# mkangquantum/quits

Hardware: AMD Instinct MI355X
Metric: decoded shots/sec + logical-error-rate, [[144,12,12]] BB code, d rounds, p=0.003 (higher is better)
Workload: dtype f32

## Files before the change

### include/quits_amd.h

```cpp
#ifndef QUITS_AMD_H
#define QUITS_AMD_H

#include <stdint.h>

#ifdef __cplusplus
extern "C" {
#endif

#define QD_OK 0
#define QD_EINVAL (-1)
#define QD_EUNSUPPORTED (-2)
#define QD_EHIP (-3)
#define QD_ECAPACITY (-4)

#define QD_BP_PRODUCT_SUM 0
#define QD_BP_MINIMUM_SUM 1
#define QD_SCHEDULE_PARALLEL 0
#define QD_SCHEDULE_SERIAL 1
#define QD_OSD_OFF 0
#define QD_OSD_0 1
#define QD_OSD_E 2
#define QD_OSD_CS 3
#define QD_LSD_0 4
#define QD_LSD_E 5
// ... 27 lines not shown
} qd_params;

int qd_version(void);
const char *qd_last_error(void);
int qd_device_count(void);

int qd_graph_create(int32_t m, int32_t n, const int32_t *row_ptr, const int32_t *col_idx, const double *priors,
                    int32_t device, qd_graph **out);
void qd_graph_destroy(qd_graph *g);
int qd_graph_info(const qd_graph *g, int32_t *info);
int qd_graph_info_ex(const qd_graph *g, int32_t *info, int32_t n_entries);

int qd_decoder_create(const qd_graph *g, const qd_params *params, qd_decoder **out);
void qd_decoder_destroy(qd_decoder *d);
int qd_decoder_info(const qd_decoder *d, int32_t *info);
#define QD_POST_NONE 0
#define QD_POST_OSD0_SR 1
#define QD_POST_OSD0_REG 2
#define QD_POST_OSD_W_OLD 3
#define QD_POST_OSD_CS_PANEL 4
#define QD_POST_LSD 5
int qd_decoder_postproc_kernel(const qd_decoder *d);
int qd_decoder_reserve(qd_decoder *d, int64_t max_batch);
int qd_decoder_set_workspace_limit(qd_decoder *d, int64_t bytes);
int qd_decoder_release_workspace(qd_decoder *d);

int qd_decode_batch(qd_decoder *d, const uint8_t *d_det, int64_t det_stride, int64_t det_offset,
                    const uint8_t *d_upd, int64_t upd_stride, int32_t upd_rows, int64_t B,
                    uint32_t *d_err_bits, int32_t *d_status, void *stream);

// ... 44 lines not shown
```

### quits_amd/_lib.py

```python
from __future__ import annotations

import ctypes as C
import os

_HERE = os.path.dirname(os.path.abspath(__file__))
LIB_PATH = os.environ.get("QUITS_AMD_LIB", os.path.join(_HERE, "lib", "libquits_amd.so"))

QD_BP = {"product_sum": 0, "ps": 0, "prod_sum": 0, "minimum_sum": 1, "min_sum": 1, "ms": 1, 0: 0, 1: 1}
QD_SCHEDULE = {"parallel": 0, "p": 0, "serial": 1, "s": 1, 0: 0, 1: 1}
QD_OSD = {"osd_off": 0, "off": 0, "osd_0": 1, "osd0": 1, "osd_e": 2, "osde": 2, "exhaustive": 2,
          "osd_cs": 3, "osdcs": 3, "combination_sweep": 3, "lsd_0": 4, "lsd_e": 5, "lsd_cs": 6, 0: 0, 1: 1, 2: 2, 3: 3, 4: 4, 5: 5, 6: 6}

STATUS_ITER_MASK = 0x3FFF
STATUS_COARSE_GRID = 1 << 14
STATUS_INEXACT = 1 << 15
STATUS_CONVERGED = 1 << 16
STATUS_OSD = 1 << 17
STATUS_INCONSISTENT = 1 << 18
STATUS_ZERO = 1 << 19


class QdParams(C.Structure):
    _fields_ = [("bp_method", C.c_int32), ("schedule", C.c_int32), ("max_iter", C.c_int32),
                ("osd_method", C.c_int32), ("osd_order", C.c_int32), ("reserved", C.c_int32),
                ("ms_scaling_factor", C.c_double)]


class QdError(RuntimeError):
    def __init__(self, code, msg):
        super().__init__("libquits_amd error %d: %s" % (code, msg))
        self.code = code


_lib = None

EXPORTS = [
    "qd_version", "qd_last_error", "qd_device_count", "qd_graph_create", "qd_graph_destroy", "qd_graph_info", "qd_graph_info_ex",
    "qd_decoder_create", "qd_decoder_info", "qd_decoder_postproc_kernel", "qd_decoder_destroy", "qd_decoder_reserve", "qd_decoder_set_workspace_limit", "qd_decoder_release_workspace", "qd_decode_batch", "qd_decode_stage", "qd_osd0_batch", "qd_decoder_failed_llr",
    "qd_decoder_set_profiling", "qd_decoder_profile", "qd_decoder_post_head_start", "qd_decoder_debug_counters", "qd_spmat_create", "qd_spmat_destroy", "qd_gf2_spmv_batch",
    "qd_unpack_bits", "qd_count_mismatch", "qd_sample_dem",
    "qd_circuit_create", "qd_circuit_destroy", "qd_circuit_info", "qd_sample_circuit",
]


def load():
    global _lib
    if _lib is not None:
        return _lib
    if not os.path.exists(LIB_PATH):
        raise RuntimeError(
            "quits_amd: %s is missing -- build it with `python -c 'import __graft_entry__ as g; g.build()'` "
            "(hipcc --offload-arch=gfx950).  There is no CPU fallback." % LIB_PATH)
    try:
# ... 4 lines not shown
    vp, i32, i64, u64 = C.c_void_p, C.c_int32, C.c_int64, C.c_uint64
    L.qd_version.restype = C.c_int
    if L.qd_version() < 104:
        raise RuntimeError("quits_amd: %s is version %d, this package needs >= 104 -- rebuild it (`python -c 'import __graft_entry__ as g; g.build()'`)"
                           % (LIB_PATH, L.qd_version()))
    L.qd_last_error.restype = C.c_char_p
    L.qd_device_count.restype = C.c_int
    L.qd_graph_create.argtypes = [i32, i32, vp, vp, vp, i32, C.POINTER(vp)]
    L.qd_graph_destroy.argtypes = [vp]
    L.qd_graph_destroy.restype = None
    L.qd_graph_info.argtypes = [vp, vp]
    L.qd_graph_info_ex.argtypes = [vp, vp, i32]
    L.qd_decoder_create.argtypes = [vp, C.POINTER(QdParams), C.POINTER(vp)]
    L.qd_decoder_info.argtypes = [vp, vp]
    L.qd_decoder_postproc_kernel.argtypes = [vp]
    L.qd_decoder_postproc_kernel.restype = C.c_int
    L.qd_decoder_destroy.argtypes = [vp]
    L.qd_decoder_destroy.restype = None
    L.qd_decoder_reserve.argtypes = [vp, i64]
    L.qd_decoder_set_workspace_limit.argtypes = [vp, i64]
    L.qd_decoder_release_workspace.argtypes = [vp]
    L.qd_decode_batch.argtypes = [vp, vp, i64, i64, vp, i64, i32, i64, vp, vp, vp]
    L.qd_decode_stage.argtypes = [vp, vp, i64, i64, vp, i64, i32, i64, vp, vp, i32, vp]
    L.qd_osd0_batch.argtypes = [vp, vp, i64, i64, vp, i64, i32, i64, vp, vp, vp, vp]
    L.qd_decoder_failed_llr.argtypes = [vp, i64, vp, vp]
    L.qd_decoder_set_profiling.argtypes = [vp, i32]
    L.qd_decoder_post_head_start.argtypes = [vp, i32, vp]
    L.qd_decoder_profile.argtypes = [vp, vp, i32]
    L.qd_decoder_debug_counters.argtypes = [vp, vp]
    L.qd_spmat_create.argtypes = [i32, i32, vp, vp, i32, C.POINTER(vp)]
# ... 28 lines not shown
```

### quits_amd/csrc/bp_scatter_edge.h

```cpp
#pragma once
#include "qd_internal.h"
#include <float.h>

__device__ __forceinline__ float qs_min_abs(float a, float b)
{
    float r;
    asm("v_min_f32 %0, %1, |%2|" : "=v"(r) : "v"(a), "v"(b));
    return r;
}
typedef uint32_t qs_u32x4 __attribute__((ext_vector_type(4)));
__device__ __forceinline__ uint4 qs_as_uint4(qs_u32x4 v) { return make_uint4(v.x, v.y, v.z, v.w); }
typedef __attribute__((address_space(3))) int32_t qs_lds_i32;
#define QS_LDS(off) ((qs_lds_i32 *)(uintptr_t)(uint32_t)(off))
#define QS_BIG 1.0e30f
#ifndef QS_PRIO
#define QS_PRIO 1
#endif

#define QS_SIGN31(sb) (((sgnw >> (sb)) & 1u) << 31)
#define QS_HP1(A_) hp ^= (uint32_t)(A_);
#define QS_HPA(A_) hpa = (uint32_t)(A_);
#define QS_HPB(A_) hp = __builtin_amdgcn_bitop3_b32(hp, hpa, (uint32_t)(A_), 0x96);
#define QS_EDGE(off, k_, sb, TAILFIX) QS_EDGE_H(off, k_, sb, TAILFIX, QS_HP1)
#define QS_EDGE_H(off, k_, sb, TAILFIX, HP)                                                                  \
    {                                                                                                        \
        const int A_ = *QS_LDS(QS_ADDR(off));                                                                \
        const float mag_ = ((uint32_t)(k_) == kold) ? s2 : s1;                                               \
        const float prev_ = __uint_as_float(QS_SIGN31(sb) | __float_as_uint(mag_));                          \
        float d_ = (float)A_ - prev_;                                                                        \
        TAILFIX(d_, k_)                                                                                      \
        const float bm_ = d_ + 1.0f;                                                                         \
        HP(A_)                                                                                               \
        neww = __builtin_amdgcn_alignbit(neww, __float_as_uint(d_), 31);                                     \
                   \
        asm("v_cmp_lt_f32 vcc, |%1|, %2\n\tv_addc_co_u32 %0, vcc, %0, %0, vcc" : "+v"(ltw) : "v"(bm_), "v"(a1) : "vcc"); \
        a2 = __builtin_amdgcn_fmed3f(a1, a2, fabsf(bm_));                                                    \
        a1 = qs_min_abs(a1, bm_);                                                                            \
    }
#define QS_NOFIX(x_, k_)
#define QS_TAILFIX(x_, k_) x_ = ((int)(k_) < dc) ? x_ : QS_BIG;

// ... 30 lines not shown
```

### quits_amd/csrc/bp_scatter_wide.hip

```cpp
#include "qd_internal.h"
#include "../../include/quits_amd.h"
#include "bp_scatter_edge.h"

#ifndef QSW_SCAT_SGPR_POS
#define QSW_SCAT_SGPR_POS 1
#endif
#ifndef QSW_GPRIO
#define QSW_GPRIO 1
#endif
#ifndef QSW_PRIO_BASE
#define QSW_PRIO_BASE 0
#endif

__device__ __forceinline__ uint4 qs_reuse4(uint4 &v) { asm volatile("" : "+v"(v.x), "+v"(v.y), "+v"(v.z), "+v"(v.w)); return v; }

template <int T, int MW, int CPL, int NSW>
__global__ void __launch_bounds__(T, MW) qd_bp_scatter_wide_kernel(BpGraphDev g, ScatGraphDev sg, DecodeArgs a, ScatArgs x)
{
    extern __shared__ __align__(16) unsigned char smem[];
    const uint32_t lds_base = (uint32_t)(uintptr_t)(__attribute__((address_space(3))) unsigned char *)smem;
    if (lds_base != 0u) __builtin_trap();
    uint32_t *outw = reinterpret_cast<uint32_t *>(smem + sg.off_out);
    int *misc = reinterpret_cast<int *>(smem + sg.off_misc);
    constexpr int NW = T / 64;
// ... 60 lines not shown
    const __amdgpu_buffer_rsrc_t adj_rsrc = __builtin_amdgcn_make_buffer_rsrc((void *)sg.adjA, 0, (g.max_rdeg_pad / 4 + 2) * m_pad * 16, 0x00020000);
    const int adj_row = m_pad * 16;
#define QS_ADJ_LOAD(row_) qs_as_uint4(__builtin_amdgcn_raw_buffer_load_b128(adj_rsrc, adj_voff, (row_) * adj_row, 0))
#ifdef QS_ABL_NOADJ
#define QS_ADJ(row_) qs_reuse4(adjc)
#define QS_ABL_ADJC uint4 adjc = QS_ADJ_LOAD(0);
#else
#define QS_ADJ(row_) QS_ADJ_LOAD(row_)
#define QS_ABL_ADJC
#endif
#ifndef QSW_PREFETCH
#define QSW_PREFETCH 1
#endif
#define QS_ADJ_FIRST qs_as_uint4(__builtin_amdgcn_raw_buffer_load_b128(adj_rsrc, cs[0] * 16, 0, 0))
    uint4 pf = QS_ADJ_FIRST;
    int t = 0, converged = 0;
    for (;;) {
        bool us = false;
#pragma unroll
        for (int j = 0; j < CPL; ++j) {
            float a1 = FLT_MAX, a2 = FLT_MAX;
            uint32_t kst = 0u;
#if QSW_GPRIO
            if (j == 0) __builtin_amdgcn_s_setprio(QSW_PRIO_BASE); else if (j == CPL - 1) __builtin_amdgcn_s_setprio((QSW_PRIO_BASE + 2) & 3); else __builtin_amdgcn_s_setprio((QSW_PRIO_BASE + 1) & 3);
#endif
            if (act[j]) {
                int dwj = dws[j];
                asm volatile("" : "+s"(dwj));
                const int trip = dwj & 0xFF, wmax = (dwj >> 8) & 0xFF, wmin = (dwj >> 16) & 0xFF, wmin4 = wmin & ~3;
                const int adj_voff = cs[j] * 16;
                QS_ABL_ADJC
                const float s1 = S1[j], s2 = S2[j];
                const uint32_t kold = KOLD[j];
                const int dc = dcs[j];
                uint32_t hp = 0u, hpa = 0u, par = 0u;
                uint32_t neg[NSW];
#pragma unroll
                for (int w = 0; w < NSW; ++w) {
                    neg[w] = 0u;
                    const int k0 = 32 * w;
                    if (k0 < trip) {
                        const uint32_t sgnw = O[j][w];
                        uint32_t neww = 0u, ltw = 0u;
                        const int kend = min(trip - k0, 32);
                        const int kplain = min(max(wmin4 - k0, 0), kend);
                        const int row0 = k0 >> 2;
                        uint4 nx = (QSW_PREFETCH && j == 0 && w == 0) ? pf : QS_ADJ(row0);
                        int kk = 0;
                        {
                            uint4 eb;
#pragma unroll 1
                            for (; kk + 8 <= kplain; kk += 8) {
                                eb = QS_ADJ(row0 + (kk >> 2) + 1);
                                {
                                    const int sb = kend - 1 - kk, k = k0 + kk;
                                    QS_EDGE_H(nx.x, k, sb, QS_NOFIX, QS_HPA) QS_EDGE_H(nx.y, k + 1, sb - 1, QS_NOFIX, QS_HPB)
                                    QS_EDGE_H(nx.z, k + 2, sb - 2, QS_NOFIX, QS_HPA) QS_EDGE_H(nx.w, k + 3, sb - 3, QS_NOFIX, QS_HPB)
                                }
                                nx = QS_ADJ(row0 + (kk >> 2) + 2);
                                {
                                    const int sb = kend - 5 - kk, k = k0 + kk + 4;
                                    QS_EDGE_H(eb.x, k, sb, QS_NOFIX, QS_HPA) QS_EDGE_H(eb.y, k + 1, sb - 1, QS_NOFIX, QS_HPB)
                                    QS_EDGE_H(eb.z, k + 2, sb - 2, QS_NOFIX, QS_HPA) QS_EDGE_H(eb.w, k + 3, sb - 3, QS_NOFIX, QS_HPB)
                                }
                            }
                        }
#pragma unroll 1
                        for (; kk < kplain; kk += 4) {
                            const uint4 e4 = nx;
                            nx = QS_ADJ(row0 + (kk >> 2) + 1);
                            const int sb = kend - 1 - kk, k = k0 + kk;
                            QS_EDGE_H(e4.x, k, sb, QS_NOFIX, QS_HPA)
                            QS_EDGE_H(e4.y, k + 1, sb - 1, QS_NOFIX, QS_HPB)
                            QS_EDGE_H(e4.z, k + 2, sb - 2, QS_NOFIX, QS_HPA)
                            QS_EDGE_H(e4.w, k + 3, sb - 3, QS_NOFIX, QS_HPB)
                        }
#define QS_TAIL_EDGE(off, q_)                                                                                     \
                            if (k + (q_) < wmin) QS_EDGE(off, k + (q_), sb - (q_), QS_NOFIX)                      \
                            else if (k + (q_) < wmax) QS_EDGE(off, k + (q_), sb - (q_), QS_TAILFIX)               \
                            else { neww <<= 1; ltw <<= 1; }
#pragma unroll 1
                        for (; kk + 4 < kend; kk += 4) {
                            const uint4 e4 = nx;
                            nx = QS_ADJ(row0 + (kk >> 2) + 1);
                            const int sb = kend - 1 - kk, k = k0 + kk;
                            QS_TAIL_EDGE(e4.x, 0) QS_TAIL_EDGE(e4.y, 1) QS_TAIL_EDGE(e4.z, 2) QS_TAIL_EDGE(e4.w, 3)
                        }
                        if (kk < kend) {
                            const int sb = kend - 1 - kk, k = k0 + kk;
                            QS_TAIL_EDGE(nx.x, 0) QS_TAIL_EDGE(nx.y, 1) QS_TAIL_EDGE(nx.z, 2) QS_TAIL_EDGE(nx.w, 3)
                        }
#undef QS_TAIL_EDGE
                        neg[w] = neww;
                        par ^= neww;
                        if (ltw) kst = (uint32_t)(k0 + kend - 1 - (int)__builtin_ctz(ltw));
                    }
                }
                const uint32_t flip = 0u - ((synd[j] ^ (uint32_t)__popc(par)) & 1u);
#pragma unroll
                for (int w = 0; w < NSW; ++w) Q[j][w] = neg[w] ^ flip;
                mx2 = fmaxf(mx2, a2);
                us = us || (((synd[j] ^ (hp >> 31)) & 1u) != 0u);
            }
            A1[j] = a1; A2[j] = a2; KST[j] = kst;
        }
#if QSW_GPRIO
        __builtin_amdgcn_s_setprio(QSW_PRIO_BASE);
#endif
        if (QSW_PREFETCH) pf = QS_ADJ_FIRST;
        {
            const unsigned long long bal = __ballot(us);
            if ((tid & 63) == 0) misc[32 + (tid >> 6)] = (bal != 0ull);
        }
        __syncthreads();
        int anyun = 0;
        {
            const int4 *f4 = reinterpret_cast<const int4 *>(misc + 32);
            for (int w = 0; w < (NW + 3) / 4; ++w) {
                const int4 v = f4[w];
                anyun |= v.x | v.y | v.z | v.w;
            }
        }
#ifndef QS_ABL_FORCE_ITERS
        if (t >= 1 && !anyun) { converged = 1; break; }
#endif
        if (t == a.max_iter) break;
        __builtin_amdgcn_s_setprio((QSW_PRIO_BASE + QS_PRIO) & 3);
#pragma unroll
        for (int j = 0; j < CPL; ++j) {
#ifdef QSW_STATS
            {
                bool same = A1[j] == S1[j] && A2[j] == S2[j] && (KST[j] == KOLD[j] || A1[j] == A2[j]);
#pragma unroll
                for (int w = 0; w < NSW; ++w) same = same && Q[j][w] == O[j][w];
                const unsigned long long ba = __ballot(act[j]), bs = __ballot(act[j] && same);
                if ((tid & 63) == 0 && ba) {
                    const int bk = min(t / 10, 4);
                    atomicAdd(&a.dbg[0], 1ull); atomicAdd(&a.dbg[2 + bk], 1ull);
                    if (bs == ba) { atomicAdd(&a.dbg[1], 1ull); atomicAdd(&a.dbg[7 + bk], 1ull); }
                    atomicAdd(&a.dbg[12], (unsigned long long)__popcll(bs)); atomicAdd(&a.dbg[13], (unsigned long long)__popcll(ba));
                }
// ... 84 lines not shown
                    const int vn = sg_ ? -dlt : dlt;
                    (void)__hip_atomic_fetch_add(QS_LDS(fixn_off), vn, __ATOMIC_RELAXED, __HIP_MEMORY_SCOPE_WORKGROUP);
                    (void)__hip_atomic_fetch_add(QS_LDS(FOFF[j]), -FVAL[j], __ATOMIC_RELAXED, __HIP_MEMORY_SCOPE_WORKGROUP);
                    FOFF[j] = fixn_off; FVAL[j] = vn;
                }
            }
            S1[j] = A1[j]; S2[j] = A2[j]; KOLD[j] = KST[j];
#pragma unroll
            for (int w = 0; w < NSW; ++w) O[j][w] = Q[j][w];
        }
        __builtin_amdgcn_s_setprio(QSW_PRIO_BASE);
        if (QSW_PREFETCH) pf = QS_ADJ_FIRST;
        __syncthreads();
        ++t;
    }
#undef QS_ADJ
#undef QS_ADJ_FIRST
#undef QS_ADJ_LOAD
#undef QS_ABL_ADJC

    {
        const int tripped = qd_block_or(!(mx2 < x.m2_limit) ? 1 : 0, misc, NW, 0);
        if (tripped) {
            if (tid == 0) {
                const int at = atomicAdd(x.recheck_count, 1);
                if (at < x.recheck_cap) x.recheck_list[at] = (int32_t)shot;
            }
            return;
        }
    }
    for (int b = tid; b < sg.nslots; b += T)
        if (*QS_LDS(cur + 4u * (uint32_t)b) < 0) {
            const uint32_t jf = sg.slot_fault[b];
            if (jf != 0xFFFFFFFFu) atomicOr(&outw[jf >> 5], 1u << (jf & 31u));
        }
    if (!converged && a.want_llr && tid == 0) misc[48] = atomicAdd(a.fail_count, 1);
    __syncthreads();
    for (int w = tid; w < g.out_words; w += T) a.err_bits[shot * g.out_words + w] = outw[w];
    if (!converged && a.want_llr) {
        const int slot = misc[48];
        float *dst = a.llr_ws + (int64_t)slot * n_pad;
        for (int k1 = tid; k1 < g.n; k1 += T) dst[k1] = (float)(*QS_LDS(cur + 4u * sg.k1_slot[k1]) + 1) * x.grid_inv;
        if (tid == 0) a.fail_list[slot] = (int32_t)shot;
    }
    if (tid == 0) a.status[shot] = t | (converged << 16) | a.status_or;
}

template <int T, int MW, int CPL, int NSW>
static hipError_t launch_scatter_wide_t(const BpGraphDev &g, const ScatGraphDev &sg, const DecodeArgs &a, const ScatArgs &x, int64_t B, hipStream_t s)
{
    auto k = qd_bp_scatter_wide_kernel<T, MW, CPL, NSW>;
    hipError_t e = hipFuncSetAttribute((const void *)k, hipFuncAttributeMaxDynamicSharedMemorySize, sg.lds_bytes);
    if (e != hipSuccess) return e;
    hipLaunchKernelGGL(k, dim3((unsigned)B), dim3(T), sg.lds_bytes, s, g, sg, a, x);
    return hipGetLastError();
}

hipError_t qd_launch_bp_scatter_wide(const BpGraphDev &g, const ScatGraphDev &sg, const DecodeArgs &a, const ScatArgs &x, int64_t B, hipStream_t s)
{
    const bool two_words = g.max_rdeg_pad <= 64;
// ... 15 lines not shown
```

### quits_amd/csrc/qd_api.hip

```cpp
#include "../../include/quits_amd.h"
#include "qd_internal.h"

#include <algorithm>
#include <cmath>
#include <cstdarg>
#include <cstdio>
#include <cstdlib>
#include <cstring>
#include <memory>
#include <numeric>
#include <vector>

#define QD_GEN_PREFIX_LDS (32 * 1024)

hipError_t qd_launch_bp(const BpGraphDev &g, const DecodeArgs &a, int64_t B, hipStream_t s);
hipError_t qd_launch_bp_scatter(const BpGraphDev &g, const ScatGraphDev &sg, const DecodeArgs &a, const ScatArgs &x, int64_t B, hipStream_t s);
hipError_t qd_launch_bp_scatter_wide(const BpGraphDev &g, const ScatGraphDev &sg, const DecodeArgs &a, const ScatArgs &x, int64_t B, hipStream_t s);
hipError_t qd_launch_bp_general(const GenGraphDev &g, const BpGraphDev &bg, const DecodeArgs &a, const GenWs &w, int bp_method,
                                int schedule, int64_t shot0, int nshots, hipStream_t s, GenStagePlan *plan);
hipError_t qd_launch_hold(const int32_t *count, int threshold, int microseconds, hipStream_t s);
int qd_bp_ps_lds_bytes(const GenGraphDev &g, int max_rdeg);
hipError_t qd_launch_bp_ps_lds(const GenGraphDev &g, const BpGraphDev &bg, const DecodeArgs &a, int64_t B, hipStream_t s);
hipError_t qd_launch_osd0(const OsdGraphDev &g, const BpGraphDev &bg, const DecodeArgs &a, int blocks_fast,
                          int blocks_full, hipStream_t s, bool handed_over = false);
int qd_osd_sr_layout(int m, int m_pad, int n, int out_words, int *off13, int *threads, int *rpt);
hipError_t qd_launch_osd0_sr(const OsdGraphDev &g, const BpGraphDev &bg, const DecodeArgs &a, int blocks, hipStream_t s);
int qd_osdcs_layout(int m, int n, int out_words, uint32_t max_wfix, int *off, int *variant, int *per_cu);
size_t qd_osdcs_ws_words(int variant);
hipError_t qd_launch_osdcs(const OsdGraphDev &g, const BpGraphDev &bg, const DecodeArgs &a, const int *off, int variant, int lds,
                           uint64_t *ws, int blocks, hipStream_t s);
size_t qd_osd_sr_ws_words(int m_pad, int mw, int threads, int rpt);
hipError_t qd_launch_lsd0(const GenGraphDev &gg, const BpGraphDev &bg, const DecodeArgs &d, uint64_t *q_ws, int blocks_alloc, int blocks,
// ... 36 lines not shown
        size_t bytes = std::max<size_t>(h.size() * sizeof(Tp), 16);
        if (hipMalloc(&d, bytes) != hipSuccess) return -1;
        ptrs.push_back(d);
        if (!h.empty() && hipMemcpy(d, h.data(), h.size() * sizeof(Tp), hipMemcpyHostToDevice) != hipSuccess) return -1;
        *out = reinterpret_cast<const Tp *>(d);
        return 0;
    }
    void release()
    {
        for (void *p : ptrs) (void)hipFree(p);
        ptrs.clear();
    }
};

struct Switches {
    bool no_scatter, scatter_cpl1, scatter_wide_t704, scatter_natural_rounds, scatter_banks_by_slot, scatter_walk_greedy, osdcs_old;
    float scatter_m2_limit;
    std::vector<int> gen_stages;
};

static Switches read_switches()
{
    auto env = [](const char *name) { return std::getenv(name); };
    Switches w{};
    w.no_scatter = env("QD_NO_SCATTER") != nullptr;
    w.scatter_cpl1 = env("QD_SCATTER_CPL1") != nullptr;
    w.scatter_wide_t704 = env("QD_SCATTER_WIDE_T704") != nullptr;
    w.scatter_natural_rounds = env("QD_SCATTER_NATURAL_ROUNDS") != nullptr;
    w.scatter_banks_by_slot = env("QD_SCATTER_BANKS_BY_SLOT") != nullptr;
    w.scatter_walk_greedy = env("QD_SCATTER_WALK_GREEDY") != nullptr;
    const char *ev = env("QD_OSDCS_OLD");
    w.osdcs_old = ev && std::atoi(ev) == 1;
    ev = env("QD_SCATTER_M2_LIMIT");
    w.scatter_m2_limit = ev ? (float)std::atof(ev) : INFINITY;
    w.gen_stages = {3, 6, 10, 14, 20, 28, 40, 56, 80, 112};
    if ((ev = env("QD_GEN_STAGES"))) {
        w.gen_stages.clear();
        for (const char *q = ev; *q;) {
            char *end = nullptr;
            const long v = std::strtol(q, &end, 10);
            if (end == q) break;
            if (v > 0) w.gen_stages.push_back((int)v);
            q = *end ? end + 1 : end;
        }
    }
    return w;
// ... 53 lines not shown
    uint64_t *cs_ws = nullptr;
    int osd_w = 0;
    int lsd_w = 0;
    uint64_t *lsd_ws = nullptr;
    int64_t gen_ws_limit = 0;
    GenWs gws{};
    GenStagePlan gsp{};
    int gen_bounds[QD_GEN_MAX_STAGES] = {0}, gen_nbounds = 0;
    int grid_k = -1, grid_kc = -1, grid_floor = 0;
    BpGraphDev bp_fine{}, bp_coarse{};
    const float *llr0_q = nullptr;
    int32_t *redo_list = nullptr;
    int redo_cap = 0;
    const int32_t *prior_g = nullptr;
    float m2_limit = 0.f;
    int32_t *recheck_list = nullptr;
    int recheck_cap = 0;
    DevAllocs mem;
    int profiling = 0;
    struct Span { int kind; hipEvent_t t0, t1; };
    std::vector<Span> ev;
    double acc_ms[4] = {0, 0, 0, 0};
};

struct qd_spmat {
    int device = 0;
    SpmatDev d{};
    DevAllocs mem;
};

// ... 119 lines not shown
                int fb = 0;
                for (int l = 0; l < 32; ++l) {
                    const bool real_lane = l < gn;
                    const int deg = real_lane ? (int)(row_ptr[chk_orig[g0 + l] + 1] - row_ptr[chk_orig[g0 + l]]) : 0;
                    if (k < deg) continue;
                    while (fb < 32 && used[fb]) ++fb;
                    const int b = fb < 32 ? fb : (l & 31);
                    if (fb < 32) used[fb]++;
                    if (g0 + l < ((m + 63) & ~63)) put(g0 + l, k, -1, b);
                }
            }
        }
    }
}

extern "C" int qd_version(void) { return 104; }
extern "C" const char *qd_last_error(void) { return g_err; }
extern "C" int qd_device_count(void)
{
    int n = 0;
    if (hipGetDeviceCount(&n) != hipSuccess) return 0;
    return n;
}

struct HostGraph {
    int m = 0, n = 0, nnz = 0, max_rdeg = 0, max_cdeg = 0, min_rdeg = 0, m_pad = 0, n_pad = 0, max_rdeg_pad = 0;
    const int32_t *row_ptr = nullptr, *col_idx = nullptr;
    const double *priors = nullptr;
    std::vector<int> rdeg, cdeg;
    std::vector<double> llr0;
    std::vector<int32_t> cp, ri, pos;
// ... 675 lines not shown
        rc |= d->mem.upload(lq, &d->llr0_q);
        if (!edge) d->bp = BP_GATHER_GRID;
        if (!edge && g->sc.ok && !env.no_scatter) {
            std::vector<int32_t> pg((size_t)g->sc.nslots, 0);
            long long mxp = 0;
            for (int j = 0; j < g->n; ++j) {
                const long long v = std::llround(std::ldexp((double)on_grid(g->h_llr0[j], d->grid_k), d->grid_k));
                pg[g->h_sc_slot[j]] = (int32_t)v - 1;
                mxp = std::max(mxp, std::llabs(v));
            }
            const long long lim = ((1ll << 23) - mxp) / std::max(1, g->max_cdeg) - 1;
            if (mxp < (1ll << 22) && lim > 0) {
                rc |= d->mem.upload(pg, &d->prior_g);
                d->m2_limit = std::min((float)lim, env.scatter_m2_limit);
                d->bp = g->sc.wide_threads ? BP_SCATTER_WIDE : BP_SCATTER;
            }
        }
        if (rc) { d->mem.release(); delete d; return fail(QD_EHIP, "device allocation failed while building the LLR grid"); }
    }
    *out = d;
    return QD_OK;
}

extern "C" int qd_decoder_info(const qd_decoder *d, int32_t *info)
{
    if (!d || !info) return fail(QD_EINVAL, "null argument");
    info[0] = d->grid_k; info[1] = d->grid_kc; info[2] = d->bp == BP_LDS_EDGE || d->bp == BP_HBM_EDGE;
    info[3] = d->bp == BP_SCATTER_WIDE ? 2 : (d->bp == BP_SCATTER ? 1 : 0);
    return QD_OK;
}

extern "C" int qd_decoder_postproc_kernel(const qd_decoder *d) { return d ? d->post : -1; }

static void free_ws(qd_decoder *d)
{
    auto dev = [](auto *&p) { if (p) (void)hipFree(p); p = nullptr; };
    auto host = [](auto *&p) { if (p) (void)hipHostFree(p); p = nullptr; };
    auto event = [](hipEvent_t &e) { if (e) (void)hipEventDestroy(e); e = nullptr; };
    dev(d->llr_ws); dev(d->fail_list); dev(d->ctr_base); dev(d->order_ws); dev(d->q_spill); dev(d->q_spill_fast); dev(d->q_spill_sr);
    dev(d->mt_ws); dev(d->cs_ws); dev(d->hard_list); dev(d->hard_list2); dev(d->redo_list); dev(d->recheck_list); dev(d->lsd_ws);
    dev(d->gws.b2c); dev(d->gws.c2b); dev(d->gws.th); dev(d->gws.pre); dev(d->gws.llr); dev(d->gws.syn); dev(d->gws.slot);
    dev(d->gsp.msg2); dev(d->gsp.syn2); dev(d->gsp.lists[0]); dev(d->gsp.lists[1]); dev(d->gsp.counts);
    host(d->host_fail); host(d->gsp.host_counts);
    event(d->fail_ready); event(d->gsp.counts_ready);
    d->gws = GenWs{}; d->gsp = GenStagePlan{};
// ... 196 lines not shown
        break;
    case BP_SCATTER_WIDE:
    case BP_SCATTER:
    case BP_GATHER_GRID: {
        int32_t *redo_count = d->fail_count + 40;
        DecodeArgs a1 = a;
        a1.s_limit = std::ldexp(1.0f, 23 - d->grid_k);
        a1.redo_list = d->redo_list; a1.redo_count = redo_count; a1.redo_cap = d->redo_cap;
        if (d->bp == BP_GATHER_GRID)
            HIP_TRY(qd_launch_bp(d->bp_fine, a1, B, s));
        else {
            int32_t *recheck_count = d->fail_count + 41;
            ScatArgs x{};
            x.prior_g = d->prior_g; x.grid_inv = std::ldexp(1.0f, -d->grid_k); x.m2_limit = d->m2_limit;
            x.recheck_list = d->recheck_list; x.recheck_count = recheck_count; x.recheck_cap = d->recheck_cap;
            if (d->bp == BP_SCATTER_WIDE) HIP_TRY(qd_launch_bp_scatter_wide(d->bp_fine, g->sc, a1, x, B, s));
            else HIP_TRY(qd_launch_bp_scatter(d->bp_fine, g->sc, a1, x, B, s));
            a1.shot_list = d->recheck_list; a1.shot_count = recheck_count;
            HIP_TRY(qd_launch_bp(d->bp_fine, a1, std::min<int64_t>(B, d->recheck_cap), s));
        }
        DecodeArgs a2 = a;
        a2.s_limit = std::ldexp(1.0f, 23 - d->grid_kc);
        a2.shot_list = d->redo_list; a2.shot_count = redo_count; a2.status_or = QD_STATUS_COARSE_GRID;
        HIP_TRY(qd_launch_bp(d->bp_coarse, a2, std::min<int64_t>(B, d->redo_cap), s));
        break;
    }
    }
    return QD_OK;
}

// ... 388 lines not shown
```

### quits_amd/csrc/qd_internal.h

```cpp
#pragma once
#include <hip/hip_runtime.h>
#include <stdint.h>

#define QD_WAVE 64
#define QD_MAX_COL_DEG 16
#define QD_MAX_ROW_DEG 255
#define QD_LDS_BYTES (160 * 1024)
#ifndef QD_SR_KWR
#define QD_SR_KWR 4
#endif
#ifndef QD_SR_WPS12
#define QD_SR_WPS12 4
#endif
#ifndef QD_SR_KWR_OF
#define QD_SR_KWR_OF(rpt) QD_SR_KWR
#endif
#ifndef QD_SR_WPS_OF
#define QD_SR_WPS_OF(rpt) ((rpt) <= 2 ? QD_SR_WPS12 : 2)
#endif
#ifndef QD_SR_TSMALL
#define QD_SR_TSMALL 512
#endif
#define QD_SR_KWR_MAX (QD_SR_KWR > 4 ? QD_SR_KWR : 4)

// ... 24 lines not shown
    const uint8_t *chk_deg;
    int offA, offB, off_out, off_bmap, off_misc, lds_bytes;
    int nslots;
    const uint32_t *slot_fault;
    const uint32_t *k1_slot;
    const int32_t *wave_map;
    int wide_threads, wide_cpl;
};
struct ScatArgs {
    const int32_t *prior_g;
    float grid_inv;
    float m2_limit;
    int32_t *recheck_list;
    int32_t *recheck_count;
    int recheck_cap;
};

#ifndef QD_GEN_D6
#define QD_GEN_D6 0
#endif
static inline int qd_gen_unroll(int max_cdeg) { return max_cdeg <= 4 ? 4 : ((QD_GEN_D6 && max_cdeg <= 6) ? 6 : (max_cdeg <= 8 ? 8 : QD_MAX_COL_DEG)); }
#ifndef QD_GEN_GS
#define QD_GEN_GS 4
#endif
struct GenGraphDev {
    int m, n, nnz, out_words;
    const int32_t *rp, *ci;
    const int32_t *cp, *ri;
    const int32_t *c2r;
    const uint16_t *erow;
// ... 177 lines not shown
```

### quits_amd/decoder/device.py

```python
from __future__ import annotations

import ctypes as C
from typing import Optional

import numpy as np

from .. import _lib
from .base import as_csr_int32


def _torch():
    import torch
    return torch


def _stream_ptr():
    torch = _torch()
    return C.c_void_p(torch.cuda.current_stream().cuda_stream)


def _ptr(t):
    return C.c_void_p(t.data_ptr())


# ... 44 lines not shown
            raise ValueError("unknown decoder option %s" % exc) from exc
        h = C.c_void_p()
        rc = L.qd_decoder_create(graph._h, C.byref(prm), C.byref(h))
        if rc == -2:
            raise NotImplementedError(L.qd_last_error().decode())
        _lib.check(rc)
        self._h = h
        self._L = L
        self.params = prm

    def info(self) -> dict:
        arr = (C.c_int32 * 4)()
        _lib.check(self._L.qd_decoder_info(self._h, arr))
        post = {0: "none", 1: "qd_osd0_sr_kernel", 2: "qd_osd0_reg_kernel", 3: "qd_osd0_reg_kernel<row form>", 4: "qd_osdcs_kernel",
                5: "qd_lsd0_kernel"}.get(int(self._L.qd_decoder_postproc_kernel(self._h)), "?")
        return {"llr_grid_bits": int(arr[0]), "llr_coarse_bits": int(arr[1]), "edge_kernel": bool(arr[2]),
                "scatter_kernel": bool(arr[3]), "scatter_wide_kernel": int(arr[3]) == 2, "post_kernel": post}

    def set_workspace_limit(self, nbytes: int):
        _lib.check(self._L.qd_decoder_set_workspace_limit(self._h, int(nbytes)))

    def release_workspace(self):
        _lib.check(self._L.qd_decoder_release_workspace(self._h))

    def reserve(self, max_batch: int):
        _lib.check(self._L.qd_decoder_reserve(self._h, int(max_batch)))

    def decode(self, det, det_offset: int = 0, upd=None, err_bits=None, status=None, stage: int = 3, stream=None):
        torch = _torch()
        assert det.is_cuda and det.dtype == torch.uint8 and det.dim() == 2 and det.stride(1) == 1
        B = det.shape[0]
        g = self.graph
# ... 179 lines not shown
```

Before: 1.533 million.

## Precompute syndrome-independent first BP check pass and thin the final iteration

When the decoder is created, a kernel runs the first check-node pass with prior-only messages, which do not depend on the syndrome. It stores per-check min1/min2, argmin and sign words in a record. Each decode then loads this record and applies a syndrome-dependent parity flip instead of walking every edge in iteration 0. The last iteration also does only a cheap hard-decision parity check instead of a full check update. This adds a decoder-time precompute and a device buffer, and correctness depends on the record exactly matching the iteration-0 walk.

Result: faster. 1.560 million, median of 6 (+1.7%).

```diff
diff --git a/include/quits_amd.h b/include/quits_amd.h
--- a/include/quits_amd.h
+++ b/include/quits_amd.h
@@ -65,6 +65,7 @@
 int qd_decoder_create(const qd_graph *g, const qd_params *params, qd_decoder **out);
 void qd_decoder_destroy(qd_decoder *d);
 int qd_decoder_info(const qd_decoder *d, int32_t *info);
+int qd_decoder_fast_start(const qd_decoder *d);
 #define QD_POST_NONE 0
 #define QD_POST_OSD0_SR 1
 #define QD_POST_OSD0_REG 2
diff --git a/quits_amd/_lib.py b/quits_amd/_lib.py
--- a/quits_amd/_lib.py
+++ b/quits_amd/_lib.py
@@ -36,7 +36,7 @@
 
 EXPORTS = [
     "qd_version", "qd_last_error", "qd_device_count", "qd_graph_create", "qd_graph_destroy", "qd_graph_info", "qd_graph_info_ex",
-    "qd_decoder_create", "qd_decoder_info", "qd_decoder_postproc_kernel", "qd_decoder_destroy", "qd_decoder_reserve", "qd_decoder_set_workspace_limit", "qd_decoder_release_workspace", "qd_decode_batch", "qd_decode_stage", "qd_osd0_batch", "qd_decoder_failed_llr",
+    "qd_decoder_create", "qd_decoder_info", "qd_decoder_fast_start", "qd_decoder_postproc_kernel", "qd_decoder_destroy", "qd_decoder_reserve", "qd_decoder_set_workspace_limit", "qd_decoder_release_workspace", "qd_decode_batch", "qd_decode_stage", "qd_osd0_batch", "qd_decoder_failed_llr",
     "qd_decoder_set_profiling", "qd_decoder_profile", "qd_decoder_post_head_start", "qd_decoder_debug_counters", "qd_spmat_create", "qd_spmat_destroy", "qd_gf2_spmv_batch",
     "qd_unpack_bits", "qd_count_mismatch", "qd_sample_dem",
     "qd_circuit_create", "qd_circuit_destroy", "qd_circuit_info", "qd_sample_circuit",
@@ -71,6 +71,9 @@
     L.qd_decoder_create.argtypes = [vp, C.POINTER(QdParams), C.POINTER(vp)]
     L.qd_decoder_info.argtypes = [vp, vp]
     L.qd_decoder_postproc_kernel.argtypes = [vp]
+    if hasattr(L, "qd_decoder_fast_start"):
+        L.qd_decoder_fast_start.argtypes = [vp]
+        L.qd_decoder_fast_start.restype = C.c_int
     L.qd_decoder_postproc_kernel.restype = C.c_int
     L.qd_decoder_destroy.argtypes = [vp]
     L.qd_decoder_destroy.restype = None
diff --git a/quits_amd/csrc/bp_scatter_edge.h b/quits_amd/csrc/bp_scatter_edge.h
--- a/quits_amd/csrc/bp_scatter_edge.h
+++ b/quits_amd/csrc/bp_scatter_edge.h
@@ -17,6 +17,7 @@
 #define QS_PRIO 1
 #endif
 
+#define QS_ACC(off) (*QS_LDS(QS_ADDR(off)))
 #define QS_SIGN31(sb) (((sgnw >> (sb)) & 1u) << 31)
 #define QS_HP1(A_) hp ^= (uint32_t)(A_);
 #define QS_HPA(A_) hpa = (uint32_t)(A_);
@@ -24,7 +25,7 @@
 #define QS_EDGE(off, k_, sb, TAILFIX) QS_EDGE_H(off, k_, sb, TAILFIX, QS_HP1)
 #define QS_EDGE_H(off, k_, sb, TAILFIX, HP)                                                                  \
     {                                                                                                        \
-        const int A_ = *QS_LDS(QS_ADDR(off));                                                                \
+        const int A_ = QS_ACC(off);                                                                          \
         const float mag_ = ((uint32_t)(k_) == kold) ? s2 : s1;                                               \
         const float prev_ = __uint_as_float(QS_SIGN31(sb) | __float_as_uint(mag_));                          \
         float d_ = (float)A_ - prev_;                                                                        \
diff --git a/quits_amd/csrc/bp_scatter_wide.hip b/quits_amd/csrc/bp_scatter_wide.hip
--- a/quits_amd/csrc/bp_scatter_wide.hip
+++ b/quits_amd/csrc/bp_scatter_wide.hip
@@ -7,6 +7,12 @@
 #endif
 #ifndef QSW_GPRIO
 #define QSW_GPRIO 1
+#endif
+#ifndef QSW_FAST_START
+#define QSW_FAST_START 1
+#endif
+#ifndef QSW_THIN_LAST
+#define QSW_THIN_LAST 1
 #endif
 #ifndef QSW_PRIO_BASE
 #define QSW_PRIO_BASE 0
@@ -98,9 +104,42 @@
 #endif
 #define QS_ADJ_FIRST qs_as_uint4(__builtin_amdgcn_raw_buffer_load_b128(adj_rsrc, cs[0] * 16, 0, 0))
     uint4 pf = QS_ADJ_FIRST;
+    const bool fast = x.first_pass != nullptr && a.max_iter >= 1;
+    bool have = false;
+    if (QSW_FAST_START && fast) {
+#pragma unroll
+        for (int j = 0; j < CPL; ++j)
+            if (act[j]) {
+                const uint4 *rp = reinterpret_cast<const uint4 *>(x.first_pass) + 2 * cs[j];
+                const uint4 r0 = rp[0], r1 = rp[1];
+                const uint32_t negw[3] = {r0.w, r1.x, r1.y};
+                const uint32_t flip = 0u - ((synd[j] ^ r1.z) & 1u);
+                A1[j] = __uint_as_float(r0.x); A2[j] = __uint_as_float(r0.y); KST[j] = r0.z;
+#pragma unroll
+                for (int w = 0; w < NSW; ++w) Q[j][w] = negw[w] ^ flip;
+                mx2 = fmaxf(mx2, A2[j]);
+            }
+        have = true;
+    }
+#define QSW_VOTE(us_, anyun_)                                                                          \
+        {                                                                                              \
+            const unsigned long long bal = __ballot(us_);                                              \
+            if ((tid & 63) == 0) misc[32 + (tid >> 6)] = (bal != 0ull);                                \
+        }                                                                                              \
+        __syncthreads();                                                                               \
+        anyun_ = 0;                                                                                    \
+        {                                                                                              \
+            const int4 *f4 = reinterpret_cast<const int4 *>(misc + 32);                                \
+            for (int w = 0; w < (NW + 3) / 4; ++w) {                                                   \
+                const int4 v = f4[w];                                                                  \
+                anyun_ |= v.x | v.y | v.z | v.w;                                                       \
+            }                                                                                          \
+        }
     int t = 0, converged = 0;
     for (;;) {
+      if (!have) {
         bool us = false;
+        if (QSW_THIN_LAST && fast && t == a.max_iter) break;
 #pragma unroll
         for (int j = 0; j < CPL; ++j) {
             float a1 = FLT_MAX, a2 = FLT_MAX;
@@ -109,77 +148,7 @@
             if (j == 0) __builtin_amdgcn_s_setprio(QSW_PRIO_BASE); else if (j == CPL - 1) __builtin_amdgcn_s_setprio((QSW_PRIO_BASE + 2) & 3); else __builtin_amdgcn_s_setprio((QSW_PRIO_BASE + 1) & 3);
 #endif
             if (act[j]) {
-                int dwj = dws[j];
-                asm volatile("" : "+s"(dwj));
-                const int trip = dwj & 0xFF, wmax = (dwj >> 8) & 0xFF, wmin = (dwj >> 16) & 0xFF, wmin4 = wmin & ~3;
-                const int adj_voff = cs[j] * 16;
-                QS_ABL_ADJC
-                const float s1 = S1[j], s2 = S2[j];
-                const uint32_t kold = KOLD[j];
-                const int dc = dcs[j];
-                uint32_t hp = 0u, hpa = 0u, par = 0u;
-                uint32_t neg[NSW];
-#pragma unroll
-                for (int w = 0; w < NSW; ++w) {
-                    neg[w] = 0u;
-                    const int k0 = 32 * w;
-                    if (k0 < trip) {
-                        const uint32_t sgnw = O[j][w];
-                        uint32_t neww = 0u, ltw = 0u;
-                        const int kend = min(trip - k0, 32);
-                        const int kplain = min(max(wmin4 - k0, 0), kend);
-                        const int row0 = k0 >> 2;
-                        uint4 nx = (QSW_PREFETCH && j == 0 && w == 0) ? pf : QS_ADJ(row0);
-                        int kk = 0;
-                        {
-                            uint4 eb;
-#pragma unroll 1
-                            for (; kk + 8 <= kplain; kk += 8) {
-                                eb = QS_ADJ(row0 + (kk >> 2) + 1);
-                                {
-                                    const int sb = kend - 1 - kk, k = k0 + kk;
-                                    QS_EDGE_H(nx.x, k, sb, QS_NOFIX, QS_HPA) QS_EDGE_H(nx.y, k + 1, sb - 1, QS_NOFIX, QS_HPB)
-                                    QS_EDGE_H(nx.z, k + 2, sb - 2, QS_NOFIX, QS_HPA) QS_EDGE_H(nx.w, k + 3, sb - 3, QS_NOFIX, QS_HPB)
-                                }
-                                nx = QS_ADJ(row0 + (kk >> 2) + 2);
-                                {
-                                    const int sb = kend - 5 - kk, k = k0 + kk + 4;
-                                    QS_EDGE_H(eb.x, k, sb, QS_NOFIX, QS_HPA) QS_EDGE_H(eb.y, k + 1, sb - 1, QS_NOFIX, QS_HPB)
-                                    QS_EDGE_H(eb.z, k + 2, sb - 2, QS_NOFIX, QS_HPA) QS_EDGE_H(eb.w, k + 3, sb - 3, QS_NOFIX, QS_HPB)
-                                }
-                            }
-                        }
-#pragma unroll 1
-                        for (; kk < kplain; kk += 4) {
-                            const uint4 e4 = nx;
-                            nx = QS_ADJ(row0 + (kk >> 2) + 1);
-                            const int sb = kend - 1 - kk, k = k0 + kk;
-                            QS_EDGE_H(e4.x, k, sb, QS_NOFIX, QS_HPA)
-                            QS_EDGE_H(e4.y, k + 1, sb - 1, QS_NOFIX, QS_HPB)
-                            QS_EDGE_H(e4.z, k + 2, sb - 2, QS_NOFIX, QS_HPA)
-                            QS_EDGE_H(e4.w, k + 3, sb - 3, QS_NOFIX, QS_HPB)
-                        }
-#define QS_TAIL_EDGE(off, q_)                                                                                     \
-                            if (k + (q_) < wmin) QS_EDGE(off, k + (q_), sb - (q_), QS_NOFIX)                      \
-                            else if (k + (q_) < wmax) QS_EDGE(off, k + (q_), sb - (q_), QS_TAILFIX)               \
-                            else { neww <<= 1; ltw <<= 1; }
-#pragma unroll 1
-                        for (; kk + 4 < kend; kk += 4) {
-                            const uint4 e4 = nx;
-                            nx = QS_ADJ(row0 + (kk >> 2) + 1);
-                            const int sb = kend - 1 - kk, k = k0 + kk;
-                            QS_TAIL_EDGE(e4.x, 0) QS_TAIL_EDGE(e4.y, 1) QS_TAIL_EDGE(e4.z, 2) QS_TAIL_EDGE(e4.w, 3)
-                        }
-                        if (kk < kend) {
-                            const int sb = kend - 1 - kk, k = k0 + kk;
-                            QS_TAIL_EDGE(nx.x, 0) QS_TAIL_EDGE(nx.y, 1) QS_TAIL_EDGE(nx.z, 2) QS_TAIL_EDGE(nx.w, 3)
-                        }
-#undef QS_TAIL_EDGE
-                        neg[w] = neww;
-                        par ^= neww;
-                        if (ltw) kst = (uint32_t)(k0 + kend - 1 - (int)__builtin_ctz(ltw));
-                    }
-                }
+#include "bp_scatter_wide_walk.inc"
                 const uint32_t flip = 0u - ((synd[j] ^ (uint32_t)__popc(par)) & 1u);
 #pragma unroll
                 for (int w = 0; w < NSW; ++w) Q[j][w] = neg[w] ^ flip;
@@ -192,23 +161,14 @@
         __builtin_amdgcn_s_setprio(QSW_PRIO_BASE);
 #endif
         if (QSW_PREFETCH) pf = QS_ADJ_FIRST;
-        {
-            const unsigned long long bal = __ballot(us);
-            if ((tid & 63) == 0) misc[32 + (tid >> 6)] = (bal != 0ull);
-        }
-        __syncthreads();
-        int anyun = 0;
-        {
-            const int4 *f4 = reinterpret_cast<const int4 *>(misc + 32);
-            for (int w = 0; w < (NW + 3) / 4; ++w) {
-                const int4 v = f4[w];
-                anyun |= v.x | v.y | v.z | v.w;
-            }
-        }
+        int anyun;
+        QSW_VOTE(us, anyun)
 #ifndef QS_ABL_FORCE_ITERS
         if (t >= 1 && !anyun) { converged = 1; break; }
 #endif
         if (t == a.max_iter) break;
+      }
+        have = false;
         __builtin_amdgcn_s_setprio((QSW_PRIO_BASE + QS_PRIO) & 3);
 #pragma unroll
         for (int j = 0; j < CPL; ++j) {
@@ -323,6 +283,45 @@
         __syncthreads();
         ++t;
     }
+    if (QSW_THIN_LAST && fast && !converged) {
+        bool us = false;
+#pragma unroll
+        for (int j = 0; j < CPL; ++j) {
+#if QSW_GPRIO
+            if (j == 0) __builtin_amdgcn_s_setprio(QSW_PRIO_BASE); else if (j == CPL - 1) __builtin_amdgcn_s_setprio((QSW_PRIO_BASE + 2) & 3); else __builtin_amdgcn_s_setprio((QSW_PRIO_BASE + 1) & 3);
+#endif
+            if (act[j]) {
+                int dwj = dws[j];
+                asm volatile("" : "+s"(dwj));
+                const int ng = (dwj & 0xFF) >> 2;
+                const int adj_voff = cs[j] * 16;
+                QS_ABL_ADJC
+                uint32_t hp = 0u, hpa = 0u;
+#define QS_HP_GROUP(e4) { QS_HPA(QS_ACC(e4.x)) QS_HPB(QS_ACC(e4.y)) QS_HPA(QS_ACC(e4.z)) QS_HPB(QS_ACC(e4.w)) }
+                uint4 nx = (QSW_PREFETCH && j == 0) ? pf : QS_ADJ(0);
+                int gi = 0;
+#pragma unroll 1
+                for (; gi + 2 <= ng; gi += 2) {
+                    const uint4 eb = QS_ADJ(gi + 1);
+                    QS_HP_GROUP(nx)
+                    nx = QS_ADJ(gi + 2);
+                    QS_HP_GROUP(eb)
+                }
+                if (gi < ng) QS_HP_GROUP(nx)
+#undef QS_HP_GROUP
+                us = us || (((synd[j] ^ (hp >> 31)) & 1u) != 0u);
+            }
+        }
+#if QSW_GPRIO
+        __builtin_amdgcn_s_setprio(QSW_PRIO_BASE);
+#endif
+        int anyun;
+        QSW_VOTE(us, anyun)
+#ifndef QS_ABL_FORCE_ITERS
+        if (!anyun) converged = 1;
+#endif
+    }
+#undef QSW_VOTE
 #undef QS_ADJ
 #undef QS_ADJ_FIRST
 #undef QS_ADJ_LOAD
@@ -353,6 +352,48 @@
         if (tid == 0) a.fail_list[slot] = (int32_t)shot;
     }
     if (tid == 0) a.status[shot] = t | (converged << 16) | a.status_or;
+}
+
+#undef QS_ACC
+#define QS_ACC(off) (prior_g[((uint32_t)(off) - (uint32_t)sg.offA) >> 2])
+#define QS_ADJ(row_) qs_as_uint4(__builtin_amdgcn_raw_buffer_load_b128(adj_rsrc, adj_voff, (row_) * adj_row, 0))
+#define QS_ABL_ADJC
+template <int NSW>
+__global__ void __launch_bounds__(64) qd_bp_first_pass_kernel(BpGraphDev g, ScatGraphDev sg, const int32_t *prior_g, uint32_t *rec)
+{
+    static_assert(NSW == 3, "the record has room for three sign words");
+    const int c = (int)blockIdx.x * 64 + (int)threadIdx.x;
+    const bool actv = c < g.m;
+    constexpr int j = 0;
+    const int cs[1] = {c}, dws[1] = {__builtin_amdgcn_readfirstlane((int)sg.deg_w[blockIdx.x])}, dcs[1] = {actv ? (int)sg.chk_deg[c] : 0};
+    const float S1[1] = {0.f}, S2[1] = {0.f};
+    const uint32_t KOLD[1] = {0xFFFFFFFFu}, O[1][NSW] = {{0u, 0u, 0u}};
+    const __amdgpu_buffer_rsrc_t adj_rsrc = __builtin_amdgcn_make_buffer_rsrc((void *)sg.adjA, 0, (g.max_rdeg_pad / 4 + 2) * g.m_pad * 16, 0x00020000);
+    const int adj_row = g.m_pad * 16;
+    const uint4 pf = qs_as_uint4(__builtin_amdgcn_raw_buffer_load_b128(adj_rsrc, c * 16, 0, 0));
+    float a1 = FLT_MAX, a2 = FLT_MAX;
+    uint32_t kst = 0u;
+    uint4 r0 = make_uint4(__float_as_uint(FLT_MAX), __float_as_uint(FLT_MAX), 0u, 0u);
+    uint4 r1 = make_uint4(0u, 0u, 0u, (uint32_t)sg.offA + (uint32_t)(sg.nslots - 32 + (int)(threadIdx.x & 31)) * 4u);
+    if (actv) {
+#include "bp_scatter_wide_walk.inc"
+        (void)hp;
+        r0 = make_uint4(__float_as_uint(a1), __float_as_uint(a2), kst, neg[0]);
+        r1 = make_uint4(neg[1], neg[2], (uint32_t)__popc(par) & 1u,
+                        __builtin_amdgcn_raw_buffer_load_b32(adj_rsrc, (int)((kst >> 2) * (uint32_t)adj_row + (kst & 3u) * 4u) + c * 16, 0, 0));
+    }
+    uint4 *out = reinterpret_cast<uint4 *>(rec) + 2 * c;
+    out[0] = r0; out[1] = r1;
+}
+#undef QS_ADJ
+#undef QS_ABL_ADJC
+#undef QS_ACC
+
+hipError_t qd_launch_bp_first_pass(const BpGraphDev &g, const ScatGraphDev &sg, const int32_t *prior_g, uint32_t *rec, hipStream_t s)
+{
+    if (g.max_rdeg_pad > 96 || g.m_pad % 64) return hipErrorInvalidValue;
+    hipLaunchKernelGGL(qd_bp_first_pass_kernel<3>, dim3((unsigned)(g.m_pad / 64)), dim3(64), 0, s, g, sg, prior_g, rec);
+    return hipGetLastError();
 }
 
 template <int T, int MW, int CPL, int NSW>
diff --git a/quits_amd/csrc/bp_scatter_wide_walk.inc b/quits_amd/csrc/bp_scatter_wide_walk.inc
--- /dev/null
+++ b/quits_amd/csrc/bp_scatter_wide_walk.inc
@@ -0,0 +1,71 @@
+                int dwj = dws[j];
+                asm volatile("" : "+s"(dwj));
+                const int trip = dwj & 0xFF, wmax = (dwj >> 8) & 0xFF, wmin = (dwj >> 16) & 0xFF, wmin4 = wmin & ~3;
+                const int adj_voff = cs[j] * 16;
+                QS_ABL_ADJC
+                const float s1 = S1[j], s2 = S2[j];
+                const uint32_t kold = KOLD[j];
+                const int dc = dcs[j];
+                uint32_t hp = 0u, hpa = 0u, par = 0u;
+                uint32_t neg[NSW];
+#pragma unroll
+                for (int w = 0; w < NSW; ++w) {
+                    neg[w] = 0u;
+                    const int k0 = 32 * w;
+                    if (k0 < trip) {
+                        const uint32_t sgnw = O[j][w];
+                        uint32_t neww = 0u, ltw = 0u;
+                        const int kend = min(trip - k0, 32);
+                        const int kplain = min(max(wmin4 - k0, 0), kend);
+                        const int row0 = k0 >> 2;
+                        uint4 nx = (QSW_PREFETCH && j == 0 && w == 0) ? pf : QS_ADJ(row0);
+                        int kk = 0;
+                        {
+                            uint4 eb;
+#pragma unroll 1
+                            for (; kk + 8 <= kplain; kk += 8) {
+                                eb = QS_ADJ(row0 + (kk >> 2) + 1);
+                                {
+                                    const int sb = kend - 1 - kk, k = k0 + kk;
+                                    QS_EDGE_H(nx.x, k, sb, QS_NOFIX, QS_HPA) QS_EDGE_H(nx.y, k + 1, sb - 1, QS_NOFIX, QS_HPB)
+                                    QS_EDGE_H(nx.z, k + 2, sb - 2, QS_NOFIX, QS_HPA) QS_EDGE_H(nx.w, k + 3, sb - 3, QS_NOFIX, QS_HPB)
+                                }
+                                nx = QS_ADJ(row0 + (kk >> 2) + 2);
+                                {
+                                    const int sb = kend - 5 - kk, k = k0 + kk + 4;
+                                    QS_EDGE_H(eb.x, k, sb, QS_NOFIX, QS_HPA) QS_EDGE_H(eb.y, k + 1, sb - 1, QS_NOFIX, QS_HPB)
+                                    QS_EDGE_H(eb.z, k + 2, sb - 2, QS_NOFIX, QS_HPA) QS_EDGE_H(eb.w, k + 3, sb - 3, QS_NOFIX, QS_HPB)
+                                }
+                            }
+                        }
+#pragma unroll 1
+                        for (; kk < kplain; kk += 4) {
+                            const uint4 e4 = nx;
+                            nx = QS_ADJ(row0 + (kk >> 2) + 1);
+                            const int sb = kend - 1 - kk, k = k0 + kk;
+                            QS_EDGE_H(e4.x, k, sb, QS_NOFIX, QS_HPA)
+                            QS_EDGE_H(e4.y, k + 1, sb - 1, QS_NOFIX, QS_HPB)
+                            QS_EDGE_H(e4.z, k + 2, sb - 2, QS_NOFIX, QS_HPA)
+                            QS_EDGE_H(e4.w, k + 3, sb - 3, QS_NOFIX, QS_HPB)
+                        }
+#define QS_TAIL_EDGE(off, q_)                                                                                     \
+                            if (k + (q_) < wmin) QS_EDGE(off, k + (q_), sb - (q_), QS_NOFIX)                      \
+                            else if (k + (q_) < wmax) QS_EDGE(off, k + (q_), sb - (q_), QS_TAILFIX)               \
+                            else { neww <<= 1; ltw <<= 1; }
+#pragma unroll 1
+                        for (; kk + 4 < kend; kk += 4) {
+                            const uint4 e4 = nx;
+                            nx = QS_ADJ(row0 + (kk >> 2) + 1);
+                            const int sb = kend - 1 - kk, k = k0 + kk;
+                            QS_TAIL_EDGE(e4.x, 0) QS_TAIL_EDGE(e4.y, 1) QS_TAIL_EDGE(e4.z, 2) QS_TAIL_EDGE(e4.w, 3)
+                        }
+                        if (kk < kend) {
+                            const int sb = kend - 1 - kk, k = k0 + kk;
+                            QS_TAIL_EDGE(nx.x, 0) QS_TAIL_EDGE(nx.y, 1) QS_TAIL_EDGE(nx.z, 2) QS_TAIL_EDGE(nx.w, 3)
+                        }
+#undef QS_TAIL_EDGE
+                        neg[w] = neww;
+                        par ^= neww;
+                        if (ltw) kst = (uint32_t)(k0 + kend - 1 - (int)__builtin_ctz(ltw));
+                    }
+                }
diff --git a/quits_amd/csrc/qd_api.hip b/quits_amd/csrc/qd_api.hip
--- a/quits_amd/csrc/qd_api.hip
+++ b/quits_amd/csrc/qd_api.hip
@@ -16,6 +16,7 @@
 hipError_t qd_launch_bp(const BpGraphDev &g, const DecodeArgs &a, int64_t B, hipStream_t s);
 hipError_t qd_launch_bp_scatter(const BpGraphDev &g, const ScatGraphDev &sg, const DecodeArgs &a, const ScatArgs &x, int64_t B, hipStream_t s);
 hipError_t qd_launch_bp_scatter_wide(const BpGraphDev &g, const ScatGraphDev &sg, const DecodeArgs &a, const ScatArgs &x, int64_t B, hipStream_t s);
+hipError_t qd_launch_bp_first_pass(const BpGraphDev &g, const ScatGraphDev &sg, const int32_t *prior_g, uint32_t *rec, hipStream_t s);
 hipError_t qd_launch_bp_general(const GenGraphDev &g, const BpGraphDev &bg, const DecodeArgs &a, const GenWs &w, int bp_method,
                                 int schedule, int64_t shot0, int nshots, hipStream_t s, GenStagePlan *plan);
 hipError_t qd_launch_hold(const int32_t *count, int threshold, int microseconds, hipStream_t s);
@@ -82,7 +83,7 @@
 };
 
 struct Switches {
-    bool no_scatter, scatter_cpl1, scatter_wide_t704, scatter_natural_rounds, scatter_banks_by_slot, scatter_walk_greedy, osdcs_old;
+    bool no_scatter, scatter_cpl1, scatter_wide_t704, scatter_natural_rounds, scatter_banks_by_slot, scatter_walk_greedy, osdcs_old, bp_no_fast_start;
     float scatter_m2_limit;
     std::vector<int> gen_stages;
 };
@@ -97,7 +98,9 @@
     w.scatter_natural_rounds = env("QD_SCATTER_NATURAL_ROUNDS") != nullptr;
     w.scatter_banks_by_slot = env("QD_SCATTER_BANKS_BY_SLOT") != nullptr;
     w.scatter_walk_greedy = env("QD_SCATTER_WALK_GREEDY") != nullptr;
-    const char *ev = env("QD_OSDCS_OLD");
+    const char *ev = env("QD_BP_NO_FAST_START");
+    w.bp_no_fast_start = ev && std::atoi(ev) == 1;
+    ev = env("QD_OSDCS_OLD");
     w.osdcs_old = ev && std::atoi(ev) == 1;
     ev = env("QD_SCATTER_M2_LIMIT");
     w.scatter_m2_limit = ev ? (float)std::atof(ev) : INFINITY;
@@ -181,6 +184,7 @@
     int redo_cap = 0;
     const int32_t *prior_g = nullptr;
     float m2_limit = 0.f;
+    const uint32_t *first_pass = nullptr;
     int32_t *recheck_list = nullptr;
     int recheck_cap = 0;
     DevAllocs mem;
@@ -330,7 +334,7 @@
     }
 }
 
-extern "C" int qd_version(void) { return 104; }
+extern "C" int qd_version(void) { return 105; }
 extern "C" const char *qd_last_error(void) { return g_err; }
 extern "C" int qd_device_count(void)
 {
@@ -1036,6 +1040,13 @@
                 rc |= d->mem.upload(pg, &d->prior_g);
                 d->m2_limit = std::min((float)lim, env.scatter_m2_limit);
                 d->bp = g->sc.wide_threads ? BP_SCATTER_WIDE : BP_SCATTER;
+                if (d->bp == BP_SCATTER_WIDE && !env.bp_no_fast_start && rc == 0) {
+                    const std::vector<uint32_t> zero((size_t)g->bp.m_pad * 8, 0u);
+                    rc |= d->mem.upload(zero, &d->first_pass);
+                    if (rc == 0 && (qd_launch_bp_first_pass(d->bp_fine, g->sc, d->prior_g, const_cast<uint32_t *>(d->first_pass), nullptr) != hipSuccess ||
+                                    hipStreamSynchronize(nullptr) != hipSuccess))
+                        rc = -1;
+                }
             }
         }
         if (rc) { d->mem.release(); delete d; return fail(QD_EHIP, "device allocation failed while building the LLR grid"); }
@@ -1051,6 +1062,8 @@
     info[3] = d->bp == BP_SCATTER_WIDE ? 2 : (d->bp == BP_SCATTER ? 1 : 0);
     return QD_OK;
 }
+
+extern "C" int qd_decoder_fast_start(const qd_decoder *d) { return d ? (d->first_pass != nullptr && d->prm.max_iter >= 1) : -1; }
 
 extern "C" int qd_decoder_postproc_kernel(const qd_decoder *d) { return d ? d->post : -1; }
 
@@ -1277,6 +1290,7 @@
             ScatArgs x{};
             x.prior_g = d->prior_g; x.grid_inv = std::ldexp(1.0f, -d->grid_k); x.m2_limit = d->m2_limit;
             x.recheck_list = d->recheck_list; x.recheck_count = recheck_count; x.recheck_cap = d->recheck_cap;
+            x.first_pass = d->first_pass;
             if (d->bp == BP_SCATTER_WIDE) HIP_TRY(qd_launch_bp_scatter_wide(d->bp_fine, g->sc, a1, x, B, s));
             else HIP_TRY(qd_launch_bp_scatter(d->bp_fine, g->sc, a1, x, B, s));
             a1.shot_list = d->recheck_list; a1.shot_count = recheck_count;
diff --git a/quits_amd/csrc/qd_internal.h b/quits_amd/csrc/qd_internal.h
--- a/quits_amd/csrc/qd_internal.h
+++ b/quits_amd/csrc/qd_internal.h
@@ -62,6 +62,7 @@
     int32_t *recheck_list;
     int32_t *recheck_count;
     int recheck_cap;
+    const uint32_t *first_pass;
 };
 
 #ifndef QD_GEN_D6
diff --git a/quits_amd/decoder/device.py b/quits_amd/decoder/device.py
--- a/quits_amd/decoder/device.py
+++ b/quits_amd/decoder/device.py
@@ -82,8 +82,9 @@
         _lib.check(self._L.qd_decoder_info(self._h, arr))
         post = {0: "none", 1: "qd_osd0_sr_kernel", 2: "qd_osd0_reg_kernel", 3: "qd_osd0_reg_kernel<row form>", 4: "qd_osdcs_kernel",
                 5: "qd_lsd0_kernel"}.get(int(self._L.qd_decoder_postproc_kernel(self._h)), "?")
+        fast = hasattr(self._L, "qd_decoder_fast_start") and int(self._L.qd_decoder_fast_start(self._h)) == 1
         return {"llr_grid_bits": int(arr[0]), "llr_coarse_bits": int(arr[1]), "edge_kernel": bool(arr[2]),
-                "scatter_kernel": bool(arr[3]), "scatter_wide_kernel": int(arr[3]) == 2, "post_kernel": post}
+                "scatter_kernel": bool(arr[3]), "scatter_wide_kernel": int(arr[3]) == 2, "bp_fast_start": fast, "post_kernel": post}
 
     def set_workspace_limit(self, nbytes: int):
         _lib.check(self._L.qd_decoder_set_workspace_limit(self._h, int(nbytes)))
```
